# Wuziyi616/LEOD

Measured on AMD Instinct MI355X. Metric: event-frames/sec/GPU (RVT-S train, Gen1 T=21) at 1/2/4/8 GPUs; mAP@0.5 parity, higher is better.
Workload: dtype fp16

## Files before the change

include/leod_hip.h:

```cpp
#ifndef LEOD_HIP_H
#define LEOD_HIP_H
#ifdef __cplusplus
extern "C" {
#endif

typedef void* leod_stream_t;

const char* leod_version(void);

int leod_set_precision(int mode);
int leod_get_precision(void);


int leod_ln_linear_fwd(const float* x, long ldx, const float* ln_w, const float* ln_b, float eps, const float* W,
                       const float* bias, float* out, float* out_act, float* stats_out, int M, int N, int K,
                       leod_stream_t stream);

int leod_linear_lsres_fwd(const float* a, const float* W, const float* bias, const float* gamma, const float* res,
                          float* out, float* tout, int M, int N, int K, leod_stream_t stream);

int leod_partition_attn_fwd(const float* qkv, float* out, float* lse, int B, int H, int W, int C, int heads, int ph,
                            int pw, int window, int qkv_bf16, leod_stream_t stream);
int leod_partition_attn_bwd(const float* qkv, const float* dout, const float* lse, float* dsum, float* dqkv, int B,
                            int H, int W, int C, int heads, int ph, int pw, int window, int qkv_bf16, int dqkv_bf16,
// ... 127 lines not shown
                       const int* strides, float ignore_label, leod_stream_t stream);
int leod_yolox_loss(const float* outputs, const float* labels, const unsigned char* fg_mask,
                    const unsigned char* ignore_mask, const int* matched_row, const float* pred_iou, const int* totals,
                    double* sums, float* losses, float* d_raw, int B, int Nmax, int nc, int nlv, const int* hs,
                    const int* ws, const int* strides, int focal, float reg_weight, float obj_weight, float cls_weight,
                    float grad_scale, leod_stream_t stream);
int leod_yolox_loss_weighted(const float* outputs, const float* labels, const unsigned char* fg_mask,
                             const unsigned char* ignore_mask, const int* matched_row, const float* pred_iou, const int* totals,
                             const float* label_w, double* wsum, double* sums, float* losses, float* d_raw, int B, int Nmax, int nc,
                             int nlv, const int* hs, const int* ws, const int* strides, int focal, float reg_weight,
                             float obj_weight, float cls_weight, float grad_scale, leod_stream_t stream);
int leod_bg_topk_ignore(const float* outputs, const float* labels, const unsigned char* fg_mask, unsigned char* ignore_mask,
                        int B, int Nmax, int A, int nc, double k, float ignore_label, leod_stream_t stream);


long leod_postprocess_nms_workspace_bytes(int B, int A);
int leod_postprocess_nms(float* pred, float* det_out, int* det_cnt, void* workspace, int B, int A, int nc, float conf_thre,
                         float nms_thre, int class_agnostic, int max_det, int vanilla_limit, leod_stream_t stream);
int leod_pseudo_filter(const float* det, const int* det_cnt, float* lab, int* lab_cnt, int B, int max_det,
                       const float* obj_thr, const float* cls_thr, int nthr, int filter_boxes, float frame_w,
                       float frame_h, leod_stream_t stream);


int leod_adamw_clip_step(float* p, float* g, float* m, float* v, long n, float lr, float beta1, float beta2, float eps,
                         float weight_decay, int step, float clip_value, float grad_scale, const float* hp_dev,
                         leod_stream_t stream);
int leod_set_weight_shadow(const float* base, long n, void* shadow16);
int leod_set_weight_shadow_f16(const float* base, void* shadow_f16);
int leod_weight_shadow_refresh(int force, leod_stream_t stream);
int leod_weight_shadow_invalidate(void);
int leod_weight_shadow_pin(int on);
int leod_act_glu_fwd(const float* p, float* h, long M, int inner, int act, int gated, leod_stream_t stream);
int leod_act_glu_bwd(const float* p, const float* dh, float* dp, long M, int inner, int act, int gated, leod_stream_t stream);
int leod_token_mask_fwd(float* x, const unsigned char* mask, const float* token, long M, int C, leod_stream_t stream);
int leod_token_mask_bwd(float* dx, const unsigned char* mask, float* dtoken, long M, int C, leod_stream_t stream);
int leod_onehot_scale(const float* g, float* out, int n, int idx, leod_stream_t stream);
int leod_set_scalars4(float* dst, float a, float b, float c, float d, leod_stream_t stream);
int leod_rows_masked_zero(void* const* tensors, const long* row_bytes, int n, const unsigned char* mask, int B, leod_stream_t stream);
int leod_copy_multi(void* const* dst, const void* const* src, const long* nbytes, int n, leod_stream_t stream);
int leod_cat2_up_fwd(const float* a, const float* b, float* out, int B, int H, int W, int Ca, int Cb, int up, leod_stream_t stream);
int leod_cat2_up_bwd(const float* dout, float* da, float* db, int B, int H, int W, int Ca, int Cb, int up, leod_stream_t stream);
int leod_rows_index_add(float* dst, const float* src, const long* idx, int nsel, long row_floats, int nrows_dst, leod_stream_t stream);
int leod_stack_hflip_u8(const void* const* frames, int T, void* out, int B, long rows_per_sample, int W, leod_stream_t stream);
int leod_voxelize_u8(const long* x, const long* y, const long* pol, const long* t, long n_events, int* counts_ws,
                     unsigned char* out, int bins, int H, int W, int count_cutoff, int fastmode, leod_stream_t stream);
int leod_mixed_density_i8(const long* x, const long* y, const long* pol, const long* t, long n_events, int* counts_ws,
                          signed char* out, int bins, int H, int W, int count_cutoff, leod_stream_t stream);

int leod_augment_u8(const unsigned char* src, unsigned char* dst, const int* params, int T, int B, int C, int H, int W,
                    leod_stream_t stream);
int leod_augment_rot_u8(const unsigned char* src, unsigned char* dst, const int* params, const float* rot, int T, int B, int C,
                        int H, int W, leod_stream_t stream);

int leod_linear_dgrad_lnbwd(const float* dy, const float* W, const float* x, const float* stats, const float* ln_w,
                            const float* dres, float* dx, float* dgamma, float* dbeta, int M, int N, int K, int dy_bf16,
                            leod_stream_t stream);

long leod_plan_create(void* hip_graph, int max_lanes);
int leod_plan_set_hoist_ranges(const long* starts, const long* bytes, int n);
int leod_plan_launch(long plan, leod_stream_t stream);
int leod_plan_rebase_input(long plan, const void* captured_base, long bytes, const void* new_base);
int leod_plan_launch_nojoin(long plan, leod_stream_t stream);
int leod_plan_join(long plan, leod_stream_t stream);
int leod_plan_info(long plan, int* info);
int leod_plan_destroy(long plan);
int leod_plan_dump(long plan, const char* path);
const char* leod_plan_last_error(void);

int leod_comm_unique_id(char* id128);
int leod_comm_init(const char* id128, int rank, int world);
int leod_comm_world(void);
int leod_comm_allreduce(void* buf, long count, int dtype, leod_stream_t stream);
int leod_comm_destroy(void);
const char* leod_comm_last_error(void);

int leod_track_filter(const float* boxes, const unsigned char* is_gt, const int* frame_idx, const int* counts, int F,
                      int img_h, int img_w, int min_track_len, double min_conf, double iou_threshold, double q,
                      unsigned char* remove, int inpaint, int* inp_frame, float* inp_box, int inp_cap, int* n_inp);

int leod_coco_eval(const float* gt_box, const int* gt_cls, const int* gt_off, const float* dt_box, const int* dt_cls,
                   const float* dt_score, const int* dt_off, int n_img, int n_cat, const double* iou_thrs, int T,
                   const double* rec_thrs, int R, double* precision, double* recall);

#ifdef __cplusplus
}
#endif
#endif
```

leod_amd/csrc/k_linear_bwd.hip:

```cpp
#include "linear_common.hpp"

LEOD_API int leod_linear_dgrad(const float* dy, long lddy, const float* kscale, const float* W, float* dx, long lddx,
                               float* dx2, long lddx2, int nsplit, const float* aux_u, float* colsum,
                               int accumulate, const float* dres, int M, int N, int K, int dy_fmt, int dx_fmt, hipStream_t stream) {
    if (!dy || !W || !dx || (N & 3) || (lddy & 3) || (dy_fmt != 0 && dy_fmt != 1) || (dx_fmt != 0 && dx_fmt != 1)) return LEOD_ERR_ARG;
    const bool dy_bf16 = dy_fmt != 0, out16 = dx_fmt != 0;
    ALRows al{}; al.x = dy; al.ld = lddy; al.kscale = kscale; al.K = N; al.fmt = dy_bf16 ? FMT_BF16 : FMT_F32;
    EpStore ep = ep_store(dx, lddx, K);
    if (out16) {
        if (leod_precision() != 1 || dx2 || colsum || accumulate || dres || aux_u || nsplit > 0 || (K & 3) || !use_gemm_lds(M, cdiv(K, 16 * pick_nt(K))))
            return LEOD_ERR_UNSUPPORTED;
        ep.out_fmt = FMT_BF16;
    }
    ep.out2 = dx2; ep.ld2 = lddx2; ep.nsplit = nsplit; ep.accumulate = accumulate; ep.colsum = colsum; ep.addsrc = dres;
    if (dres && (nsplit > 0 || accumulate)) return LEOD_ERR_ARG;
    if (aux_u) { ep.act = ACT_MUL_GELU_GRAD; ep.aux = aux_u; ep.ldaux = K; }
    const int nt = pick_nt(K);
    int rc = LEOD_OK;
    if (!dy_bf16 && !out16 && !dx2 && !colsum && !accumulate && !dres && lddy == N && lddx == K && nsplit <= 0) {
        if (!kscale && !aux_u && use_rowstream_narrow(M, N, K))
            return launch_rowstream_narrow<1>(dy, W, nullptr, nullptr, nullptr, dx, M, N, stream);
        if (const int slab = rowstream_slab(M, K, N)) {
            if (N == 48 && slab == 12) return launch_rowstream_dgrad<3, 12>(dy, lddy, kscale, W, aux_u, dx, M, K, stream);
            if (N == 96 && slab == 8) return launch_rowstream_dgrad<6, 8>(dy, lddy, kscale, W, aux_u, dx, M, K, stream);
            if (N == 64 && slab == 8) return launch_rowstream_dgrad<4, 8>(dy, lddy, kscale, W, aux_u, dx, M, K, stream);
        }
    }
    if (use_gemm_lds(M, cdiv(K, 16 * nt))) {
        DISPATCH_NT(nt, { BLTrans bl{W, (long)K, K, NT}; rc = launch_gemm_lds<NT>(al, bl, ep, M, N, cdiv(K, 16 * NT), stream); });
        return rc;
    }
    DISPATCH_NT(nt, { BLTrans bl{W, (long)K, K, NT}; rc = launch_gemm16<NT>(al, bl, ep, M, N, cdiv(K, 16 * NT), stream); });
    return rc;
}

LEOD_API int leod_linear_dgrad_lnbwd(const float* dy, const float* W, const float* x, const float* stats, const float* ln_w,
                                     const float* dres, float* dx, float* dgamma, float* dbeta, int M, int N, int K, int dy_bf16,
                                     hipStream_t stream) {
    if (!dy || !W || !x || !stats || !ln_w || !dx || !dgamma || !dbeta) return LEOD_ERR_ARG;
    if (dy_bf16 && use_rowstream_narrow96(M, N, K)) {
        const dim3 g96(min(cdiv(cdiv(M, 16), 8), 256));
        if (N == 384) hipLaunchKernelGGL((rowstream_narrow_kernel<24, 2, 1, 2, 6>), g96, dim3(512), 0, stream, dy, W, nullptr, ln_w, dres, dx, M, x, stats, dgamma, dbeta);
        else hipLaunchKernelGGL((rowstream_narrow_kernel<18, 2, 1, 2, 6>), g96, dim3(512), 0, stream, dy, W, nullptr, ln_w, dres, dx, M, x, stats, dgamma, dbeta);
        return leod_launch_status();
    }
    if (!use_rowstream_narrow(M, N, K)) return LEOD_ERR_UNSUPPORTED;
    const int grid = min(cdiv(cdiv(M, 16), 4), 256 * 2);
    if (dy_bf16) {
        if (leod_precision() != 1) return LEOD_ERR_ARG;
        if (N == 192) hipLaunchKernelGGL((rowstream_narrow_kernel<12, 2, 1, 2>), dim3(grid), dim3(256), 0, stream, dy, W, nullptr, ln_w, dres, dx, M, x, stats, dgamma, dbeta);
        else hipLaunchKernelGGL((rowstream_narrow_kernel<9, 2, 1, 2>), dim3(grid), dim3(256), 0, stream, dy, W, nullptr, ln_w, dres, dx, M, x, stats, dgamma, dbeta);
        return leod_launch_status();
    }
    if (leod_precision() == 1) {
        if (N == 192) hipLaunchKernelGGL((rowstream_narrow_kernel<12, 2, 1>), dim3(grid), dim3(256), 0, stream, dy, W, nullptr, ln_w, dres, dx, M, x, stats, dgamma, dbeta);
        else hipLaunchKernelGGL((rowstream_narrow_kernel<9, 2, 1>), dim3(grid), dim3(256), 0, stream, dy, W, nullptr, ln_w, dres, dx, M, x, stats, dgamma, dbeta);
        return leod_launch_status();
    }
    if (N == 192) hipLaunchKernelGGL((rowstream_narrow_kernel<12, 2>), dim3(grid), dim3(256), 0, stream, dy, W, nullptr, ln_w, dres, dx, M, x, stats, dgamma, dbeta);
    else hipLaunchKernelGGL((rowstream_narrow_kernel<9, 2>), dim3(grid), dim3(256), 0, stream, dy, W, nullptr, ln_w, dres, dx, M, x, stats, dgamma, dbeta);
    return leod_launch_status();
}

LEOD_API int leod_linear_dgrad_gelu16(const float* dy, const float* kscale, const float* W, const void* u16, void* dx,
                                      int M, int N, int K, int out_bf16, hipStream_t stream) {
    if (!dy || !W || !u16 || !dx || leod_precision() != 1) return LEOD_ERR_ARG;
    const int slab = rowstream_slab(M, K, N);
    if (!slab) {
        const int nt = pick_nt(K);
        if ((N & 3) || (K & 3) || !use_gemm_lds(M, cdiv(K, 16 * nt))) return LEOD_ERR_UNSUPPORTED;
        ALRows al{}; al.x = dy; al.ld = N; al.kscale = kscale; al.K = N;
        EpStore ep = ep_store(reinterpret_cast<float*>(dx), K, K);
        ep.act = ACT_MUL_GELU_GRAD; ep.aux = reinterpret_cast<const float*>(u16); ep.ldaux = K; ep.aux_fmt = FMT_F16PRE; ep.out_fmt = out_bf16 ? FMT_BF16 : FMT_F32;
        int rc = LEOD_OK;
        DISPATCH_NT(nt, { BLTrans bl{W, (long)K, K, NT}; rc = launch_gemm_lds<NT>(al, bl, ep, M, N, cdiv(K, 16 * NT), stream); });
        return rc;
    }
    const int slabs = K / (16 * slab);
    const int gx = min(cdiv(cdiv(M, 16), 4), max(8, (256 * 2 / slabs) & ~7));
    float* aux = reinterpret_cast<float*>(const_cast<void*>(u16));
#define DG16_CASE(KCV, NTTV)                                                                                                         \
    if (N == 16 * KCV && slab == NTTV) {                                                                                             \
        if (out_bf16) hipLaunchKernelGGL((rowstream48_kernel<KCV, NTTV, false, false, 2, 1, true, 1>), dim3(gx, slabs), dim3(256), 0, stream, \
                                         dy, (long)N, nullptr, kscale, nullptr, 0.f, W, nullptr, reinterpret_cast<float*>(dx), aux, M, K);          \
        else hipLaunchKernelGGL((rowstream48_kernel<KCV, NTTV, false, false, 2, 1, true>), dim3(gx, slabs), dim3(256), 0, stream, dy, (long)N, \
                                nullptr, kscale, nullptr, 0.f, W, nullptr, reinterpret_cast<float*>(dx), aux, M, K);                              \
        return leod_launch_status();                                                                                                 \
    }
    DG16_CASE(3, 12) DG16_CASE(6, 8) DG16_CASE(4, 8)
#undef DG16_CASE
    return LEOD_ERR_UNSUPPORTED;
}
```

leod_amd/csrc/linear_common.hpp:

```cpp
#pragma once
#include <type_traits>

#define LEOD_SHADOW_KERNELS 1
#include "gemm16.hpp"

static inline int pick_nt(int N) {
    int best = 1; long bestpad = 1L << 60;
    for (int nt = 4; nt >= 1; --nt) {
        const long pad = (long)cdiv(N, 16 * nt) * 16 * nt;
        if (pad < bestpad) { bestpad = pad; best = nt; }
    }
    return best;
}

#define DISPATCH_NT(NTV, ...)                                          \
    switch (NTV) {                                                     \
        case 1: { constexpr int NT = 1; __VA_ARGS__; } break;          \
        case 2: { constexpr int NT = 2; __VA_ARGS__; } break;          \
        case 3: { constexpr int NT = 3; __VA_ARGS__; } break;          \
        default: { constexpr int NT = 4; __VA_ARGS__; } break;         \
    }


static inline EpStore ep_store(float* out, long ld, int N) {
// ... 138 lines not shown
            *reinterpret_cast<f4*>(out + row * Ntot + n) = v;
            if (ACT) {
                f4 ge;
#pragma unroll
                for (int j = 0; j < 4; ++j) ge[j] = gelu_erf(v[j]);
                *reinterpret_cast<f4*>(out2 + row * Ntot + n) = ge;
            }
        };
#pragma unroll
        for (int g = 0; g < NG; ++g) {
            const int nt_g = NTT - 4 * g >= 4 ? 4 : NTT - 4 * g;
            asm volatile("s_waitcnt lgkmcnt(0)" ::: "memory");
            __builtin_amdgcn_wave_barrier();
#pragma unroll
            for (int t = 4 * g; t < NTT && t < 4 * g + 4; ++t)
#pragma unroll
                for (int r = 0; r < 4; ++r) so[(4 * q + r) * LDO + 16 * (t - 4 * g) + i] = acc[t][r];
            asm volatile("s_waitcnt lgkmcnt(0)" ::: "memory");
            __builtin_amdgcn_wave_barrier();
            if (nt_g == 4) {
#pragma unroll
                for (int p = 0; p < 4; ++p) {
                    const int lr = q + 4 * p;
                    emit(row0 + lr, 64 * g + 4 * i, *reinterpret_cast<const f4*>(&so[lr * LDO + 4 * i]) + bv[g], ug[DG == 2 ? 4 * g + p : 0]);
                }
            } else {
                const int lr = lane >> 2, c4 = lane & 3;
                const f4 b4 = {__shfl(bv[g][0], c4, 64), __shfl(bv[g][1], c4, 64), __shfl(bv[g][2], c4, 64), __shfl(bv[g][3], c4, 64)};
                emit(row0 + lr, 64 * g + 4 * c4, *reinterpret_cast<const f4*>(&so[lr * LDO + 4 * c4]) + b4, ug[DG == 2 ? 4 * g : 0]);
            }
        }
    };
    static_assert(NTT % 4 == 0 || NTT % 4 == 1, "remainder groups of 2 or 3 column tiles are not laid out");
    const int nfull = M / 16;
    int tile = blockIdx.x * 4 + wave;
    Frag f0, f1, f2;
    load(f0, tile);
    load(f1, tile + stride);
    const std::true_type full{};
    while (true) {
        load(f2, tile + 2 * stride);
        if (tile >= nfull) break;
        compute(f0, tile, full); tile += stride;
        load(f0, tile + 2 * stride);
        if (tile >= nfull) { f0 = f1; break; }
        compute(f1, tile, full); tile += stride;
        load(f1, tile + 2 * stride);
        if (tile >= nfull) { f0 = f2; break; }
        compute(f2, tile, full); tile += stride;
    }
    if (tile == nfull && (M & 15)) compute(f0, tile, std::false_type{});
}

template <int KC, int MODE, int BF = 0, int AF = 0, int NTN = 3>
__global__ __launch_bounds__(NTN == 3 ? 256 : 512, NTN == 3 ? 2 : 1) void rowstream_narrow_kernel(const float* __restrict__ x, const float* __restrict__ W,
                                                                  const float* __restrict__ bias, const float* __restrict__ gamma,
                                                                  const float* __restrict__ res, float* __restrict__ out, int M,
                                                                  const float* __restrict__ xin = nullptr,
                                                                  const float* __restrict__ stats = nullptr,
                                                                  float* __restrict__ dgamma = nullptr, float* __restrict__ dbeta = nullptr) {
    constexpr int K = 16 * KC, LD = K + 8, N = 16 * NTN, LDO = N + 4, NWV = NTN == 3 ? 4 : 8, NTHR = 64 * NWV, F4R = N / 4;
    __shared__ __attribute__((aligned(16))) float sW[BF ? (N * LD) / 2 : N * LD];
    __shared__ __attribute__((aligned(16))) float sO[NWV][16 * LDO];
    unsigned short* sWh = reinterpret_cast<unsigned short*>(sW);
    const int tid = threadIdx.x, lane = tid & 63, wave = tid >> 6;
    const int i = lane & 15, q = lane >> 4;
    if (MODE == 0) {
        for (int e = tid; e < N * (K / 4); e += NTHR) {
            const int n = e / (K / 4), k4 = (e - n * (K / 4)) * 4;
            if constexpr (BF) *reinterpret_cast<s4*>(&sWh[n * LD + k4]) = pack16_raw<BF>(ld4(W + (long)n * K + k4));
            else *reinterpret_cast<f4*>(&sW[n * LD + k4]) = ld4(W + (long)n * K + k4);
        }
    } else {
        for (int e = tid; e < K * (N / 4); e += NTHR) {
            const int k = e / (N / 4), n4 = (e - k * (N / 4)) * 4;
            const f4 w = ld4(W + (long)k * N + n4);
            if constexpr (BF) {
                const s4 wh = pack16_raw<BF>(w);
#pragma unroll
                for (int j = 0; j < 4; ++j) sWh[(n4 + j) * LD + k] = (unsigned short)wh[j];
            } else {
#pragma unroll
                for (int j = 0; j < 4; ++j) sW[(n4 + j) * LD + k] = w[j];
            }
        }
    }
    int lr[NTN], c4[NTN];
    f4 b4[NTN], g4[NTN];
#pragma unroll
    for (int p = 0; p < NTN; ++p) {
        const int idx = 64 * p + lane;
        lr[p] = idx / F4R; c4[p] = idx - lr[p] * F4R;
        b4[p] = (MODE == 0 && bias) ? ld4(bias + 4 * c4[p]) : zero4();
        g4[p] = (MODE == 0 && gamma) ? ld4(gamma + 4 * c4[p]) : f4{1.f, 1.f, 1.f, 1.f};
    }
    float lnw[NTN], agam[NTN], abet[NTN];
#pragma unroll
    for (int t = 0; t < NTN; ++t) { lnw[t] = 1.f; agam[t] = 0.f; abet[t] = 0.f; }
    if (MODE == 2) {
#pragma unroll
        for (int t = 0; t < NTN; ++t) lnw[t] = gamma[16 * t + i];
    }
    __syncthreads();
    const int stride = gridDim.x * NWV;
    float* so = sO[wave];
    typedef typename std::conditional<AF != 0, s4, f4>::type AFrag;
    struct Frag { AFrag a[KC]; };
    auto load = [&](Frag& f, int tile) {
        const long row = min((long)tile * 16 + i, (long)M - 1);
        if constexpr (AF) {
            const unsigned short* p = reinterpret_cast<const unsigned short*>(x) + row * K + 4 * q;
#pragma unroll
            for (int c = 0; c < KC; ++c) f.a[c] = *reinterpret_cast<const s4*>(p + 16 * c);
        } else {
            const float* p = x + row * K + 4 * q;
#pragma unroll
            for (int c = 0; c < KC; ++c) f.a[c] = ld4(p + 16 * c);
        }
    };
    auto compute = [&](const Frag& f, int tile, auto full_tag) {
        constexpr bool FULL = decltype(full_tag)::value;
        const long row0 = (long)tile * 16;
        f4 r4[NTN];
        if (MODE == 0 || (MODE == 2 && res)) {
#pragma unroll
            for (int p = 0; p < NTN; ++p) {
                const long row = FULL ? row0 + lr[p] : min(row0 + lr[p], (long)M - 1);
                r4[p] = ld4(res + row * N + 4 * c4[p]);
            }
        }
        float xi[NTN][4], mean[4], rstd[4];
        if (MODE == 2) {
#pragma unroll
            for (int r = 0; r < 4; ++r) {
                const long row = FULL ? row0 + 4 * q + r : min(row0 + 4 * q + r, (long)M - 1);
                const float2 st = *reinterpret_cast<const float2*>(stats + 2 * row);
                mean[r] = st.x; rstd[r] = st.y;
#pragma unroll
                for (int t = 0; t < NTN; ++t) xi[t][r] = xin[row * N + 16 * t + i];
            }
        }
        f4 acc[NTN];
#pragma unroll
        for (int t = 0; t < NTN; ++t) acc[t] = zero4();
#pragma unroll
        for (int c = 0; c < KC; ++c) {
            if constexpr (BF) {
                s4 pa;
                if constexpr (AF == 2) pa = f.a[c];
                else if constexpr (AF == 1) {
                    f4 u = unpack_h16(f.a[c]);
#pragma unroll
                    for (int j = 0; j < 4; ++j) u[j] = gelu_erf(u[j]);
                    pa = pack16<BF>(u);
                } else pa = pack16<BF>(f.a[c]);
#pragma unroll
                for (int t = 0; t < NTN; ++t)
                    acc[t] = mfma16_16<BF>(pa, *reinterpret_cast<const s4*>(&sWh[(16 * t + i) * LD + 16 * c + 4 * q]), acc[t]);
            } else if constexpr (AF == 0) {
#pragma unroll
            for (int t = 0; t < NTN; ++t) {
                const f4 b = *reinterpret_cast<const f4*>(&sW[(16 * t + i) * LD + 16 * c + 4 * q]);
#pragma unroll
                for (int j = 0; j < 4; ++j) acc[t] = mfma16(f.a[c][j], b[j], acc[t]);
            }
            }
        }
        if (MODE == 2) {
#pragma unroll
            for (int r = 0; r < 4; ++r) {
                const bool live = FULL || row0 + 4 * q + r < M;
                float s1 = 0.f, s2 = 0.f, xh[NTN], gw[NTN];
#pragma unroll
                for (int t = 0; t < NTN; ++t) {
                    const float dn = live ? acc[t][r] : 0.f;
                    xh[t] = (xi[t][r] - mean[r]) * rstd[r];
                    gw[t] = dn * lnw[t];
                    agam[t] += dn * xh[t]; abet[t] += dn;
                    s1 += gw[t]; s2 += gw[t] * xh[t];
                }
                s1 = row16_sum(s1) * (1.0f / N);
                s2 = row16_sum(s2) * (1.0f / N);
#pragma unroll
                for (int t = 0; t < NTN; ++t) acc[t][r] = (gw[t] - s1 - xh[t] * s2) * rstd[r];
            }
        }
        asm volatile("s_waitcnt lgkmcnt(0)" ::: "memory");
        __builtin_amdgcn_wave_barrier();
#pragma unroll
        for (int t = 0; t < NTN; ++t)
#pragma unroll
            for (int r = 0; r < 4; ++r) so[(4 * q + r) * LDO + 16 * t + i] = acc[t][r];
        asm volatile("s_waitcnt lgkmcnt(0)" ::: "memory");
        __builtin_amdgcn_wave_barrier();
#pragma unroll
        for (int p = 0; p < NTN; ++p) {
            f4 v = *reinterpret_cast<const f4*>(&so[lr[p] * LDO + 4 * c4[p]]);
            if (MODE == 0) v = r4[p] + g4[p] * (v + b4[p]);
            if (MODE == 2 && res) v = v + r4[p];
            if (FULL || row0 + lr[p] < M) *reinterpret_cast<f4*>(out + (row0 + lr[p]) * N + 4 * c4[p]) = v;
        }
    };
    const int nfull = M / 16;
    int tile = blockIdx.x * NWV + wave;
    const std::true_type full{};
    if constexpr (NTN == 3) {
        Frag f0, f1, f2;
        load(f0, tile);
        load(f1, tile + stride);
        while (true) {
            load(f2, tile + 2 * stride);
            if (tile >= nfull) break;
            compute(f0, tile, full); tile += stride;
            load(f0, tile + 2 * stride);
            if (tile >= nfull) { f0 = f1; break; }
            compute(f1, tile, full); tile += stride;
            load(f1, tile + 2 * stride);
            if (tile >= nfull) { f0 = f2; break; }
            compute(f2, tile, full); tile += stride;
        }
        if (tile == nfull && (M & 15)) compute(f0, tile, std::false_type{});
    } else {
        Frag f0, f1;
        load(f0, tile);
        while (true) {
            load(f1, tile + stride);
            if (tile >= nfull) break;
            compute(f0, tile, full); tile += stride;
            load(f0, tile + stride);
            if (tile >= nfull) { f0 = f1; break; }
            compute(f1, tile, full); tile += stride;
        }
        if (tile == nfull && (M & 15)) compute(f0, tile, std::false_type{});
    }
    if (MODE == 2) {
#pragma unroll
        for (int t = 0; t < NTN; ++t) {
            float a = agam[t], b = abet[t];
            a += __shfl_xor(a, 16, 64); a += __shfl_xor(a, 32, 64);
            b += __shfl_xor(b, 16, 64); b += __shfl_xor(b, 32, 64);
            if (q == 0) { atomicAdd(dgamma + 16 * t + i, a); atomicAdd(dbeta + 16 * t + i, b); }
        }
    }
}
static inline bool use_rowstream_narrow(int M, int Kc, int Nout) {
    return M >= 16384 && Nout == 48 && (Kc == 144 || Kc == 192);
}
static inline bool use_rowstream_narrow96(int M, int Kc, int Nout) {
    return leod_precision() == 1 && M >= 16384 && Nout == 96 && (Kc == 288 || Kc == 384);
}
template <int MODE>
static int launch_rowstream_narrow(const float* x, const float* W, const float* bias, const float* gamma, const float* res,
// ... 47 lines not shown
```

leod_amd/functions.py:

```python
import os
from typing import Optional, Tuple

import torch
from torch.autograd import Function

from . import ops
from .comm import NativeComm

_SYNC_BN = {'group': None, 'world_size': 1, 'force': False, 'images': None, 'n_collectives': 0}



class WgradSide:
    active = False
    hold_main = False
    streams = {}
    used = set()
    keep = []

    @classmethod
    def side_of(cls, main):
        key = main.cuda_stream
        st = cls.streams.get(key)
        if st is None:
# ... 152 lines not shown
            return
        if not PlanRecorder.split(exchange):
            exchange()


def sync_bn_begin(n_images: int, device) -> None:
    if not _sync_bn_on():
        _SYNC_BN['images'] = None
        return
    images = torch.full((1,), float(n_images), dtype=torch.float64, device=device)
    _allreduce_stats(images)
    _SYNC_BN['images'] = images


def flush_bn_counters(module: torch.nn.Module) -> None:
    bufs, incs = [], []
    for m in module.modules():
        n = getattr(m, 'bn_calls_pending', 0)
        if n and hasattr(m, 'bn'):
            bufs.append(m.bn.num_batches_tracked)
            incs.append(n)
            m.bn_calls_pending = 0
    if bufs:
        if len(set(incs)) == 1:
            torch._foreach_add_(bufs, incs[0])
        else:
            for b, n in zip(bufs, incs):
                b += n


def grad_buf(p: torch.nn.Parameter) -> torch.Tensor:
    if p.grad is None:
        p.grad = torch.zeros_like(p, memory_format=torch.contiguous_format)
    return p.grad


def to_nhwc(t: torch.Tensor) -> torch.Tensor:
    v = t.permute(0, 2, 3, 1)
    return v if v.is_contiguous() else v.contiguous()


def as_nchw(t_nhwc: torch.Tensor) -> torch.Tensor:
    return t_nhwc.permute(0, 3, 1, 2)


def _cont(t: Optional[torch.Tensor]) -> Optional[torch.Tensor]:
    return None if t is None else (t if t.is_contiguous() else t.contiguous())


def _rows(t: Optional[torch.Tensor]) -> Optional[torch.Tensor]:
    return None if t is None else (t if ops.row_stride(t, t.shape[-1]) else t.contiguous())


class ConvLNFn(Function):

    @staticmethod
    def forward(ctx, mod, x, conv_w, ln_w, ln_b, is_stem: bool, stride: int, padded_hw):
        need = any(ctx.needs_input_grad)
        if is_stem:
            z = ops.stem_conv_fwd(x, conv_w, padded_hw, stride, mod.conv.padding[0])
        else:
            z = ops.conv_nhwc_fwd(x, conv_w, None, stride=stride)
        y, stats = ops.layernorm_fwd(z, ln_w, ln_b, want_stats=need)
        ctx.mod, ctx.is_stem, ctx.stride, ctx.padded_hw = mod, is_stem, stride, padded_hw
        ctx.save_for_backward(x, z, stats, conv_w, ln_w)
        return y

    @staticmethod
    def backward(ctx, dy):
        x, z, stats, conv_w, ln_w = ctx.saved_tensors
        mod = ctx.mod
        if mod.norm.weight is not None:
            dlw, dlb = grad_buf(mod.norm.weight), grad_buf(mod.norm.bias)
        else:
            dlw, dlb = torch.zeros_like(ln_w), torch.zeros_like(ln_w)
        dz = ops.layernorm_bwd(_cont(dy), z, stats, ln_w, None, dlw, dlb)
        dx = None
        if ctx.is_stem:
            ops.stem_conv_wgrad(dz, x, grad_buf(mod.conv.weight), ctx.padded_hw, ctx.stride, mod.conv.padding[0])
        else:
            with _wgrad_side(dz, x):
                ops.conv_nhwc_wgrad(dz, x, grad_buf(mod.conv.weight), None, stride=ctx.stride)
            if ctx.needs_input_grad[1]:
                dx = ops.conv_nhwc_dgrad(dz, conv_w, x.shape, stride=ctx.stride)
        return None, dx, None, None, None, None, None, None


class AttnBlockFn(Function):

    @staticmethod
    def forward(ctx, mod, x, *params):
        need = any(ctx.needs_input_grad)
        (n1w, n1b, qkv_w, qkv_b, proj_w, proj_b, g1, n2w, n2b, fc1_w, fc1_b, fc2_w, fc2_b, g2) = params
        heads, part, window = mod.self_attn.num_heads, mod.partition_size, mod.partition_window
        q16 = ops.partition_attn_16bit_ok(x.shape[0], x.shape[1], x.shape[2], x.shape[3], heads, part)
        qkv, _, st1 = ops.ln_linear_fwd(x, n1w, n1b, qkv_w, qkv_b, want_stats=need or q16, out_bf16=q16)
        o16 = q16 and ops.attn_block_o16_ok(x.shape[0], x.shape[1], x.shape[2], x.shape[3], heads, part)
        o, lse = ops.partition_attn_fwd(qkv, heads, part, window, want_lse=need, out_bf16=o16)
        y, _ = ops.linear_lsres_fwd(o, proj_w, proj_b, g1, x, want_t=False, a_gelu=False)
        fused = ops.mlp_fwd_fused(y, n2w, n2b, fc1_w, fc1_b, fc2_w, fc2_b, g2, want_saved=need)
        if fused is not None:
            z, u, st2 = fused
            h = None
        else:
            u, h, st2 = ops.ln_linear_fwd(y, n2w, n2b, fc1_w, fc1_b, want_act=True, want_stats=True)
            z, _ = ops.linear_lsres_fwd(h if h is not None else u, fc2_w, fc2_b, g2, y, want_t=False, a_gelu=h is None)
        if need:
            ctx.mod = mod
            ctx.u16 = h is None
            ctx.save_for_backward(x, qkv, st1, o, lse, y, u, u if h is None else h, st2, *params)
        return z

    @staticmethod
    def backward(ctx, dz):
        (x, qkv, st1, o, lse, y, u, h, st2,
         n1w, n1b, qkv_w, qkv_b, proj_w, proj_b, g1, n2w, n2b, fc1_w, fc1_b, fc2_w, fc2_b, g2) = ctx.saved_tensors
        mod = ctx.mod
        sa, mlp = mod.self_attn, mod.mlp
        heads, part, window = sa.num_heads, mod.partition_size, mod.partition_window
        dz = _cont(dz)
        fused = None
        if ctx.u16:
            fused = ops.mlp_bwd_dgrad_fused(dz, y, st2, n2w, n2b, fc1_w, fc1_b, fc2_w, g2, grad_buf(mod.norm2.weight), grad_buf(mod.norm2.bias))
        if fused is not None:
            dy, du = fused
        else:
            du = ops.linear_dgrad(dz, fc2_w, kscale=g2, aux_u=u)
            dy = ops.linear_dgrad_ln_bwd(du, fc1_w, y, st2, n2w, dz, grad_buf(mod.norm2.weight), grad_buf(mod.norm2.bias))
        do = ops.linear_dgrad(dy, proj_w, kscale=g1, out_bf16=o.dtype is not torch.float32)
        dqkv = ops.partition_attn_bwd(qkv, do, lse, heads, part, window)
        with _wgrad_side(dz, h, du, y, st2, dy, o, dqkv, x, st1):
            grouped = ops.attn_block_wgrads(dz, h, ctx.u16, du, y, st2, n2w, n2b, dy, o, dqkv, x, st1, n1w, n1b,
                                            (fc2_w, fc2_b, g2, grad_buf(mlp.net[2].weight), grad_buf(mlp.net[2].bias), grad_buf(mod.ls2.gamma)),
                                            (grad_buf(mlp.net[0][0].weight), grad_buf(mlp.net[0][0].bias)),
                                            (proj_w, proj_b, g1, grad_buf(sa.proj.weight), grad_buf(sa.proj.bias), grad_buf(mod.ls1.gamma)),
                                            (grad_buf(sa.qkv.weight), grad_buf(sa.qkv.bias)))
            if not grouped:
                ops.layerscale_linear_wgrad(dz, h, fc2_w, fc2_b, g2, grad_buf(mlp.net[2].weight), grad_buf(mlp.net[2].bias),
                                            grad_buf(mod.ls2.gamma), h_gelu=ctx.u16)
                ops.linear_wgrad(du, y, grad_buf(mlp.net[0][0].weight), grad_buf(mlp.net[0][0].bias), stats=st2, ln_w=n2w, ln_b=n2b)
                ops.layerscale_linear_wgrad(dy, o, proj_w, proj_b, g1, grad_buf(sa.proj.weight), grad_buf(sa.proj.bias),
                                            grad_buf(mod.ls1.gamma), h_gelu=False)
                if n1w is not None:
                    ops.linear_wgrad(dqkv, x, grad_buf(sa.qkv.weight), grad_buf(sa.qkv.bias), stats=st1, ln_w=n1w, ln_b=n1b)
                else:
                    ops.linear_wgrad(dqkv, x, grad_buf(sa.qkv.weight), grad_buf(sa.qkv.bias))
        if n1w is not None:
            dx = ops.linear_dgrad_ln_bwd(dqkv, qkv_w, x, st1, n1w, dy, grad_buf(mod.norm1.weight), grad_buf(mod.norm1.bias))
        else:
            dx = ops.linear_dgrad(dqkv, qkv_w, dres=dy)
        return (None, dx) + (None,) * 14


class ConvLSTMFn(Function):

    @staticmethod
    def forward(ctx, mod, x, h_prev, c_prev, w, b):
        need = any(ctx.needs_input_grad)
        C = x.shape[-1]
        h, c, gates = ops.convlstm_fwd(x, h_prev, c_prev, w.view(4 * C, 2 * C), b, want_gates=need)
        if need:
            ctx.mod = mod
            ctx.set_materialize_grads(False)
            ctx.save_for_backward(x, h_prev, c_prev, c, gates, w)
        return h, c

    @staticmethod
    def backward(ctx, dh, dc):
        x, h_prev, c_prev, c, gates, w = ctx.saved_tensors
        mod = ctx.mod
        C = x.shape[-1]
        dgates, dc_prev = ops.convlstm_gates_bwd(_cont(dh), _cont(dc), gates, c_prev, c, want_dc_prev=ctx.needs_input_grad[3])
        with _wgrad_side(dgates, x, h_prev):
            ops.linear_wgrad(dgates, x, grad_buf(mod.conv1x1.weight).view(4 * C, 2 * C), grad_buf(mod.conv1x1.bias), x2=h_prev)
        dx, dh_prev = ops.linear_dgrad(dgates, w.view(4 * C, 2 * C), split=C)
        dx = dx.view(x.shape)
        dh_prev = dh_prev.view(x.shape) if ctx.needs_input_grad[2] else None
        return None, dx, dh_prev, dc_prev, None, None


class DepthwiseConvFn(Function):

    @staticmethod
    def forward(ctx, conv, x, w, b, lo: int, hi: int):
        wv, bv = w[lo:hi], (b[lo:hi] if b is not None else None)
        y = ops.conv_nhwc_fwd(x, wv, bv, stride=1)
        if any(ctx.needs_input_grad):
            ctx.conv, ctx.lohi = conv, (lo, hi)
            ctx.save_for_backward(x, w)
        return y

    @staticmethod
    def backward(ctx, dy):
        x, w = ctx.saved_tensors
        lo, hi = ctx.lohi
        dy = _cont(dy)
        db = grad_buf(ctx.conv.bias)[lo:hi] if ctx.conv.bias is not None else None
        with _wgrad_side(dy, x):
            ops.conv_nhwc_wgrad(dy, x, grad_buf(ctx.conv.weight)[lo:hi], db, stride=1)
        dx = ops.conv_nhwc_dgrad(dy, w[lo:hi], x.shape, stride=1) if ctx.needs_input_grad[1] else None
        return None, dx, None, None, None, None


# ... 438 lines not shown
```

leod_amd/ops.py:

```python
from typing import Optional, Sequence, Tuple

import ctypes

import torch

from ._lib import lib, check, LeodHipError, DevPtr

F32 = torch.float32


_LIB = None


def _l():
    global _LIB
    if _LIB is None:
        _LIB = lib()
    return _LIB


try:
    _raw_stream = torch._C._cuda_getCurrentRawStream
except AttributeError:
    _raw_stream = None
# ... 445 lines not shown
    if rc == -3:
        if ev is not None:
            _PROBE.cancel('linear_wgrad')
        return False
    check(rc, 'linear_wgrad_group')
    if ev is not None:
        ev.record()
    return True


def attn_block_wgrads(dz, h, h_gelu, du, y, st2, n2w, n2b, dy, o, dqkv, x, st1, n1w, n1b, fc2, fc1, proj, qkv) -> bool:
    W2, b2, g2, dW2, db2, dg2 = fc2
    Wp, bp, g1, dWp, dbp, dg1 = proj
    (N2, K2), (Np, Kp) = W2.shape, Wp.shape
    if not is_16bit() or dz.numel() // N2 < 8192:
        return False
    scratch = StatArena.zeros((N2 * K2 + N2 + Np * Kp + Np,), dz.device, torch.float32)
    G2, s2 = scratch[:N2 * K2].view(N2, K2), scratch[N2 * K2:N2 * K2 + N2]
    off = N2 * K2 + N2
    Gp, sp = scratch[off:off + Np * Kp].view(Np, Kp), scratch[off + Np * Kp:]
    probs = [dict(dy=dz, x=h, dW=G2, dbias=s2, gelu=bool(h_gelu)),
             dict(dy=du, x=y, dW=fc1[0], dbias=fc1[1], stats=st2, ln_w=n2w, ln_b=n2b),
             dict(dy=dy, x=o, dW=Gp, dbias=sp),
             dict(dy=dqkv, x=x, dW=qkv[0], dbias=qkv[1], stats=st1 if n1w is not None else None, ln_w=n1w, ln_b=n1b)]
    if not linear_wgrad_group(probs):
        return False
    check(_l().leod_layerscale_finalize(_p(W2), _p(b2), _p(g2), _p(G2), _p(s2), _p(dW2), _p(db2), _p(dg2), N2, K2, _stream()), 'layerscale_finalize')
    check(_l().leod_layerscale_finalize(_p(Wp), _p(bp), _p(g1), _p(Gp), _p(sp), _p(dWp), _p(dbp), _p(dg1), Np, Kp, _stream()), 'layerscale_finalize')
    return True


def layernorm_fwd(x, w, b, want_stats=False, eps=1e-5):
    for t, n in ((x, 'x'), (w, 'w'), (b, 'b')):
        _ck(t, name=n)
    C = x.shape[-1]
    M = x.numel() // C
    y = _empty(x.shape, x)
    stats = _empty((M, 2), x) if want_stats else None
    check(_l().leod_layernorm_fwd(_p(x), _p(w), _p(b), _p(y), _p(stats), M, C, eps, _stream()), 'layernorm_fwd')
    return y, stats


def layernorm_bwd(dn, x, stats, w, dres, dw, db, eps=1e-5):
    for t, n in ((dn, 'dn'), (x, 'x'), (stats, 'stats'), (w, 'w'), (dres, 'dres'), (dw, 'dw'), (db, 'db')):
        _ck(t, name=n)
    C = x.shape[-1]
    M = x.numel() // C
    dx = _empty(x.shape, x)
    check(_l().leod_layernorm_bwd(_p(dn), _p(x), _p(stats), _p(w), _p(dres), _p(dx), _p(dw), _p(db), M, C, eps,
                                   _stream()), 'layernorm_bwd')
    return dx


def linear_dgrad_ln_bwd(dy, W, x, stats, ln_w, dres, dw, db, eps=1e-5):
    dy16 = dy.dtype is torch.bfloat16
    _ck(dy, torch.bfloat16 if dy16 else F32, 'dy')
    for t, n in ((W, 'W'), (x, 'x'), (stats, 'stats'), (ln_w, 'ln_w'), (dres, 'dres'), (dw, 'dw'), (db, 'db')):
        _ck(t, name=n)
    N, K = W.shape
    M = dy.numel() // N
    dx = _empty(x.shape, x)
    rc = _l().leod_linear_dgrad_lnbwd(_p(dy), _p(W), _p(x), _p(stats), _p(ln_w), _p(dres), _p(dx), _p(dw), _p(db), M, N, K,
                                      1 if dy16 else 0, _stream())
    if rc == -3:
        return layernorm_bwd(linear_dgrad(dy, W), x, stats, ln_w, dres, dw, db, eps)
    check(rc, 'linear_dgrad_lnbwd')
    return dx


def layerscale_bwd(dz, t, gamma, dgamma):
    for tt, n in ((dz, 'dz'), (t, 't'), (gamma, 'gamma'), (dgamma, 'dgamma')):
        _ck(tt, name=n)
    C = dz.shape[-1]
    M = dz.numel() // C
    dt = _empty(dz.shape, dz)
    check(_l().leod_layerscale_bwd(_p(dz), _p(t), _p(gamma), _p(dt), _p(dgamma), M, C, _stream()), 'layerscale_bwd')
    return dt


def layerscale_linear_wgrad(dz, h, W, b, gamma, dW, db, dgamma, h_gelu=None):
    N, K = W.shape
    scratch = StatArena.zeros((N * K + N,), dz.device, torch.float32)
    G, s = scratch[:N * K].view(N, K), scratch[N * K:]
    linear_wgrad(dz, h, G, s, x_gelu=h_gelu)
    check(_l().leod_layerscale_finalize(_p(W), _p(b), _p(gamma), _p(G), _p(s), _p(dW), _p(db), _p(dgamma), N, K, _stream()),
          'layerscale_finalize')


def _out_hw(H, W, ks, stride, pad):
    return (H + 2 * pad - ks) // stride + 1, (W + 2 * pad - ks) // stride + 1


def stem_conv_fwd(x_nchw, w, padded_hw, stride, pad):
    if x_nchw.dtype not in (torch.uint8, F32):
        raise LeodHipError(f'stem input must be uint8 or float32, got {x_nchw.dtype}')
    _ck(x_nchw, x_nchw.dtype, 'x')
    _ck(w, name='w')
    B, Cin, H, W = x_nchw.shape
    N, ks = w.shape[0], w.shape[-1]
    Ho, Wo = _out_hw(padded_hw[0], padded_hw[1], ks, stride, pad)
    y = torch.empty((B, Ho, Wo, N), dtype=F32, device=x_nchw.device)
    check(_l().leod_stem_conv_fwd(_p(x_nchw), 1 if x_nchw.dtype == torch.uint8 else 0, _p(w), _p(y), B, Cin, H, W,
                                   padded_hw[0], padded_hw[1], N, ks, stride, pad, _stream()), 'stem_conv_fwd')
    return y


def stem_conv_wgrad(dy, x_nchw, dw, padded_hw, stride, pad):
    _ck(dy, name='dy')
    _ck(x_nchw, x_nchw.dtype, 'x')
    _ck(dw, name='dw')
    B, Cin, H, W = x_nchw.shape
    N, ks = dw.shape[0], dw.shape[-1]
    check(_l().leod_stem_conv_wgrad(_p(dy), _p(x_nchw), 1 if x_nchw.dtype == torch.uint8 else 0, _p(dw), B, Cin, H, W,
                                     padded_hw[0], padded_hw[1], N, ks, stride, pad, _stream()), 'stem_conv_wgrad')


BF16_GRADS = True
STAT_REPLICAS = 32

# ... 868 lines not shown
```

Before: 11420.

## Fuse downsample LayerNorm backward into following attention block's qkv dgrad

Records the conv-LN forward state on its output tensor so the next attention block, which lacks its own norm1, can run the fused linear-dgrad + LayerNorm-backward kernel with the residual added before the LN backward (new res-first mode). The ConvLN backward then reuses the precomputed dz when the incoming gradient is the same buffer, or applies a correction for extra gradient contributions otherwise. This aims to remove a separate layernorm_bwd pass and a full-size intermediate write/read. It adds cross-Function coupling through tensor attributes, which is fragile if the gradient reaching the ConvLN differs from the one the fused kernel saw.

```diff
diff --git a/include/leod_hip.h b/include/leod_hip.h
--- a/include/leod_hip.h
+++ b/include/leod_hip.h
@@ -203,9 +203,10 @@
 int leod_augment_rot_u8(const unsigned char* src, unsigned char* dst, const int* params, const float* rot, int T, int B, int C,
                         int H, int W, leod_stream_t stream);
 
+int leod_linear_dgrad_lnbwd_supported(int M, int N, int K, int dy_bf16);
 int leod_linear_dgrad_lnbwd(const float* dy, const float* W, const float* x, const float* stats, const float* ln_w,
                             const float* dres, float* dx, float* dgamma, float* dbeta, int M, int N, int K, int dy_bf16,
-                            leod_stream_t stream);
+                            int res_mode, leod_stream_t stream);
 
 long leod_plan_create(void* hip_graph, int max_lanes);
 int leod_plan_set_hoist_ranges(const long* starts, const long* bytes, int n);
diff --git a/leod_amd/csrc/k_linear_bwd.hip b/leod_amd/csrc/k_linear_bwd.hip
--- a/leod_amd/csrc/k_linear_bwd.hip
+++ b/leod_amd/csrc/k_linear_bwd.hip
@@ -34,32 +34,43 @@
     return rc;
 }
 
+LEOD_API int leod_linear_dgrad_lnbwd_supported(int M, int N, int K, int dy_bf16) {
+    if (dy_bf16 && use_rowstream_narrow96(M, N, K)) return 1;
+    return use_rowstream_narrow(M, N, K) && (!dy_bf16 || leod_precision() == 1);
+}
+
 LEOD_API int leod_linear_dgrad_lnbwd(const float* dy, const float* W, const float* x, const float* stats, const float* ln_w,
                                      const float* dres, float* dx, float* dgamma, float* dbeta, int M, int N, int K, int dy_bf16,
-                                     hipStream_t stream) {
-    if (!dy || !W || !x || !stats || !ln_w || !dx || !dgamma || !dbeta) return LEOD_ERR_ARG;
+                                     int res_mode, hipStream_t stream) {
+    if (!dy || !W || !x || !stats || !ln_w || !dx || !dgamma || !dbeta || (res_mode != 0 && res_mode != 1)) return LEOD_ERR_ARG;
+    const bool rf = res_mode == 1 && dres;
+#define LNBWD_LAUNCH(KCV, BFV, AFV, NTNV, GRID, NTHR)                                                                               \
+    do {                                                                                                                            \
+        if (rf) hipLaunchKernelGGL((rowstream_narrow_kernel<KCV, 2, BFV, AFV, NTNV, 1>), GRID, dim3(NTHR), 0, stream, dy, W, nullptr, ln_w,  \
+                                   dres, dx, M, x, stats, dgamma, dbeta);                                                           \
+        else hipLaunchKernelGGL((rowstream_narrow_kernel<KCV, 2, BFV, AFV, NTNV, 0>), GRID, dim3(NTHR), 0, stream, dy, W, nullptr, ln_w,    \
+                                dres, dx, M, x, stats, dgamma, dbeta);                                                              \
+        return leod_launch_status();                                                                                                \
+    } while (0)
     if (dy_bf16 && use_rowstream_narrow96(M, N, K)) {
         const dim3 g96(min(cdiv(cdiv(M, 16), 8), 256));
-        if (N == 384) hipLaunchKernelGGL((rowstream_narrow_kernel<24, 2, 1, 2, 6>), g96, dim3(512), 0, stream, dy, W, nullptr, ln_w, dres, dx, M, x, stats, dgamma, dbeta);
-        else hipLaunchKernelGGL((rowstream_narrow_kernel<18, 2, 1, 2, 6>), g96, dim3(512), 0, stream, dy, W, nullptr, ln_w, dres, dx, M, x, stats, dgamma, dbeta);
-        return leod_launch_status();
+        if (N == 384) LNBWD_LAUNCH(24, 1, 2, 6, g96, 512);
+        LNBWD_LAUNCH(18, 1, 2, 6, g96, 512);
     }
     if (!use_rowstream_narrow(M, N, K)) return LEOD_ERR_UNSUPPORTED;
-    const int grid = min(cdiv(cdiv(M, 16), 4), 256 * 2);
+    const dim3 grid(min(cdiv(cdiv(M, 16), 4), 256 * 2));
     if (dy_bf16) {
         if (leod_precision() != 1) return LEOD_ERR_ARG;
-        if (N == 192) hipLaunchKernelGGL((rowstream_narrow_kernel<12, 2, 1, 2>), dim3(grid), dim3(256), 0, stream, dy, W, nullptr, ln_w, dres, dx, M, x, stats, dgamma, dbeta);
-        else hipLaunchKernelGGL((rowstream_narrow_kernel<9, 2, 1, 2>), dim3(grid), dim3(256), 0, stream, dy, W, nullptr, ln_w, dres, dx, M, x, stats, dgamma, dbeta);
-        return leod_launch_status();
+        if (N == 192) LNBWD_LAUNCH(12, 1, 2, 3, grid, 256);
+        LNBWD_LAUNCH(9, 1, 2, 3, grid, 256);
     }
     if (leod_precision() == 1) {
-        if (N == 192) hipLaunchKernelGGL((rowstream_narrow_kernel<12, 2, 1>), dim3(grid), dim3(256), 0, stream, dy, W, nullptr, ln_w, dres, dx, M, x, stats, dgamma, dbeta);
-        else hipLaunchKernelGGL((rowstream_narrow_kernel<9, 2, 1>), dim3(grid), dim3(256), 0, stream, dy, W, nullptr, ln_w, dres, dx, M, x, stats, dgamma, dbeta);
-        return leod_launch_status();
+        if (N == 192) LNBWD_LAUNCH(12, 1, 0, 3, grid, 256);
+        LNBWD_LAUNCH(9, 1, 0, 3, grid, 256);
     }
-    if (N == 192) hipLaunchKernelGGL((rowstream_narrow_kernel<12, 2>), dim3(grid), dim3(256), 0, stream, dy, W, nullptr, ln_w, dres, dx, M, x, stats, dgamma, dbeta);
-    else hipLaunchKernelGGL((rowstream_narrow_kernel<9, 2>), dim3(grid), dim3(256), 0, stream, dy, W, nullptr, ln_w, dres, dx, M, x, stats, dgamma, dbeta);
-    return leod_launch_status();
+    if (N == 192) LNBWD_LAUNCH(12, 0, 0, 3, grid, 256);
+    LNBWD_LAUNCH(9, 0, 0, 3, grid, 256);
+#undef LNBWD_LAUNCH
 }
 
 LEOD_API int leod_linear_dgrad_gelu16(const float* dy, const float* kscale, const float* W, const void* u16, void* dx,
diff --git a/leod_amd/csrc/linear_common.hpp b/leod_amd/csrc/linear_common.hpp
--- a/leod_amd/csrc/linear_common.hpp
+++ b/leod_amd/csrc/linear_common.hpp
@@ -214,13 +214,14 @@
     if (tile == nfull && (M & 15)) compute(f0, tile, std::false_type{});
 }
 
-template <int KC, int MODE, int BF = 0, int AF = 0, int NTN = 3>
+template <int KC, int MODE, int BF = 0, int AF = 0, int NTN = 3, int RF = 0>
 __global__ __launch_bounds__(NTN == 3 ? 256 : 512, NTN == 3 ? 2 : 1) void rowstream_narrow_kernel(const float* __restrict__ x, const float* __restrict__ W,
                                                                   const float* __restrict__ bias, const float* __restrict__ gamma,
                                                                   const float* __restrict__ res, float* __restrict__ out, int M,
                                                                   const float* __restrict__ xin = nullptr,
                                                                   const float* __restrict__ stats = nullptr,
                                                                   float* __restrict__ dgamma = nullptr, float* __restrict__ dbeta = nullptr) {
+    static_assert(RF == 0 || MODE == 2, "residual-first is a mode of the LayerNorm-backward epilogue");
     constexpr int K = 16 * KC, LD = K + 8, N = 16 * NTN, LDO = N + 4, NWV = NTN == 3 ? 4 : 8, NTHR = 64 * NWV, F4R = N / 4;
     __shared__ __attribute__((aligned(16))) float sW[BF ? (N * LD) / 2 : N * LD];
     __shared__ __attribute__((aligned(16))) float sO[NWV][16 * LDO];
@@ -284,7 +285,7 @@
         constexpr bool FULL = decltype(full_tag)::value;
         const long row0 = (long)tile * 16;
         f4 r4[NTN];
-        if (MODE == 0 || (MODE == 2 && res)) {
+        if (MODE == 0 || (MODE == 2 && !RF && res)) {
 #pragma unroll
             for (int p = 0; p < NTN; ++p) {
                 const long row = FULL ? row0 + lr[p] : min(row0 + lr[p], (long)M - 1);
@@ -305,6 +306,14 @@
         f4 acc[NTN];
 #pragma unroll
         for (int t = 0; t < NTN; ++t) acc[t] = zero4();
+        if constexpr (RF != 0) {
+#pragma unroll
+            for (int r = 0; r < 4; ++r) {
+                const long row = FULL ? row0 + 4 * q + r : min(row0 + 4 * q + r, (long)M - 1);
+#pragma unroll
+                for (int t = 0; t < NTN; ++t) acc[t][r] = res[row * N + 16 * t + i];
+            }
+        }
 #pragma unroll
         for (int c = 0; c < KC; ++c) {
             if constexpr (BF) {
@@ -359,7 +368,7 @@
         for (int p = 0; p < NTN; ++p) {
             f4 v = *reinterpret_cast<const f4*>(&so[lr[p] * LDO + 4 * c4[p]]);
             if (MODE == 0) v = r4[p] + g4[p] * (v + b4[p]);
-            if (MODE == 2 && res) v = v + r4[p];
+            if (MODE == 2 && !RF && res) v = v + r4[p];
             if (FULL || row0 + lr[p] < M) *reinterpret_cast<f4*>(out + (row0 + lr[p]) * N + 4 * c4[p]) = v;
         }
     };
diff --git a/leod_amd/functions.py b/leod_amd/functions.py
--- a/leod_amd/functions.py
+++ b/leod_amd/functions.py
@@ -228,6 +228,21 @@
     return None if t is None else (t if ops.row_stride(t, t.shape[-1]) else t.contiguous())
 
 
+class LNRecord:
+    __slots__ = ('mod', 'z', 'stats', 'ln_w', 'claimed', 'dz')
+    taken = 0
+    corrected = 0
+
+    def __init__(self, mod, z, stats, ln_w):
+        self.mod, self.z, self.stats, self.ln_w, self.claimed, self.dz = mod, z, stats, ln_w, False, None
+
+    def clear(self):
+        self.mod = self.z = self.stats = self.ln_w = self.dz = None
+
+
+LN_RECORDS = True
+
+
 class ConvLNFn(Function):
 
     @staticmethod
@@ -240,6 +255,9 @@
         y, stats = ops.layernorm_fwd(z, ln_w, ln_b, want_stats=need)
         ctx.mod, ctx.is_stem, ctx.stride, ctx.padded_hw = mod, is_stem, stride, padded_hw
         ctx.save_for_backward(x, z, stats, conv_w, ln_w)
+        ctx.rec = None
+        if need and LN_RECORDS and mod.norm.weight is not None:
+            ctx.rec = y._ln_record = LNRecord(mod, z, stats, ln_w)
         return y
 
     @staticmethod
@@ -250,7 +268,18 @@
             dlw, dlb = grad_buf(mod.norm.weight), grad_buf(mod.norm.bias)
         else:
             dlw, dlb = torch.zeros_like(ln_w), torch.zeros_like(ln_w)
-        dz = ops.layernorm_bwd(_cont(dy), z, stats, ln_w, None, dlw, dlb)
+        rec, ctx.rec = ctx.rec, None
+        fused = rec.dz if rec is not None else None
+        if rec is not None:
+            rec.clear()
+        if fused is None:
+            dz = ops.layernorm_bwd(_cont(dy), z, stats, ln_w, None, dlw, dlb)
+        elif dy.data_ptr() == fused.data_ptr() and dy.shape == fused.shape:
+            dz = fused
+            LNRecord.taken += 1
+        else:
+            dz = fused + ops.layernorm_bwd(_cont(dy) - fused, z, stats, ln_w, None, dlw, dlb)
+            LNRecord.corrected += 1
         dx = None
         if ctx.is_stem:
             ops.stem_conv_wgrad(dz, x, grad_buf(mod.conv.weight), ctx.padded_hw, ctx.stride, mod.conv.padding[0])
@@ -284,6 +313,11 @@
         if need:
             ctx.mod = mod
             ctx.u16 = h is None
+            rec = getattr(x, '_ln_record', None) if n1w is None and ctx.needs_input_grad[1] else None
+            ctx.ln_rec = None
+            if rec is not None and not rec.claimed and rec.z is not None and rec.z.shape == x.shape:
+                rec.claimed = True
+                ctx.ln_rec = rec
             ctx.save_for_backward(x, qkv, st1, o, lse, y, u, u if h is None else h, st2, *params)
         return z
 
@@ -324,7 +358,13 @@
         if n1w is not None:
             dx = ops.linear_dgrad_ln_bwd(dqkv, qkv_w, x, st1, n1w, dy, grad_buf(mod.norm1.weight), grad_buf(mod.norm1.bias))
         else:
-            dx = ops.linear_dgrad(dqkv, qkv_w, dres=dy)
+            rec, ctx.ln_rec = ctx.ln_rec, None
+            if rec is not None and rec.z is not None:
+                nrm = rec.mod.norm
+                dx = rec.dz = ops.linear_dgrad_ln_bwd(dqkv, qkv_w, rec.z, rec.stats, rec.ln_w, dy, grad_buf(nrm.weight), grad_buf(nrm.bias),
+                                                      res_first=True)
+            else:
+                dx = ops.linear_dgrad(dqkv, qkv_w, dres=dy)
         return (None, dx) + (None,) * 14
 
 
diff --git a/leod_amd/ops.py b/leod_amd/ops.py
--- a/leod_amd/ops.py
+++ b/leod_amd/ops.py
@@ -521,19 +521,24 @@
     return dx
 
 
-def linear_dgrad_ln_bwd(dy, W, x, stats, ln_w, dres, dw, db, eps=1e-5):
+def linear_dgrad_ln_bwd_supported(M, N, K, dy16) -> bool:
+    return bool(_l().leod_linear_dgrad_lnbwd_supported(int(M), int(N), int(K), 1 if dy16 else 0))
+
+
+def linear_dgrad_ln_bwd(dy, W, x, stats, ln_w, dres, dw, db, eps=1e-5, res_first=False):
     dy16 = dy.dtype is torch.bfloat16
     _ck(dy, torch.bfloat16 if dy16 else F32, 'dy')
     for t, n in ((W, 'W'), (x, 'x'), (stats, 'stats'), (ln_w, 'ln_w'), (dres, 'dres'), (dw, 'dw'), (db, 'db')):
         _ck(t, name=n)
     N, K = W.shape
     M = dy.numel() // N
+    if not linear_dgrad_ln_bwd_supported(M, N, K, dy16):
+        if res_first:
+            return layernorm_bwd(linear_dgrad(dy, W, dres=dres), x, stats, ln_w, None, dw, db, eps)
+        return layernorm_bwd(linear_dgrad(dy, W), x, stats, ln_w, dres, dw, db, eps)
     dx = _empty(x.shape, x)
-    rc = _l().leod_linear_dgrad_lnbwd(_p(dy), _p(W), _p(x), _p(stats), _p(ln_w), _p(dres), _p(dx), _p(dw), _p(db), M, N, K,
-                                      1 if dy16 else 0, _stream())
-    if rc == -3:
-        return layernorm_bwd(linear_dgrad(dy, W), x, stats, ln_w, dres, dw, db, eps)
-    check(rc, 'linear_dgrad_lnbwd')
+    check(_l().leod_linear_dgrad_lnbwd(_p(dy), _p(W), _p(x), _p(stats), _p(ln_w), _p(dres), _p(dx), _p(dw), _p(db), M, N, K,
+                                       1 if dy16 else 0, 1 if res_first and dres is not None else 0, _stream()), 'linear_dgrad_lnbwd')
     return dx
 
 
```

Result: no change. 11480 (median of 6 runs) (+0.6%).
